# danaesavi/SocialMedia-TextImage-Classification-AuxLosses

Measured on AMD Instinct MI355X. Metric: posts/sec (fwd+bwd) Bernice+ViT-B/16 attn-fusion, bs=64, higher is better.
Workload: dtype bf16; 1 GPU; BASELINE config 2: Bernice+ViT-B/16, attention fusion, no aux loss, bs=64/GPU; step=full train step: fwd + loss + bwd + grad exchange + AdamW + weight refresh, posts_per_gpu=64, image=224, vocab=250002, parallelism=dp1, weights=random-init at true shapes

## Files before the change

### socialmedia-textimage-classification-auxlosses_amd/csrc/engine.hip

```cpp
#include <string>
#include <vector>
#include <cstdlib>
#include <cstdio>
#include "mmhip_common.h"
#include "mmhip_host.h"

using namespace mmhip;

namespace {

struct LayerOff {
    size_t qkv_w, qkv_b, ao_w, ao_b, ln1_w, ln1_b, fc1_w, fc1_b, fc2_w, fc2_b, ln2_w, ln2_b, begin, end;
};
struct LayerW16 {
    size_t qkv, ao, fc1, fc2, qkvT, aoT, fc1T, fc2T;
};
struct TextAct {
    size_t qkv, ctx, pre1, a1, u, h, pre2, out, mean1, rstd1, mean2, rstd2, lse;
    size_t a1p, outp;
};

}

struct mmhip_engine {
// ... 31 lines not shown
    int B = 0, T = 0, Bt = 0; bool itm = false, train_mode = false, fwd_done = false, bwd_begun = false;
    bool skip_itc = false, itc_done = false;
    uint64_t seed = 0;
    size_t ws_base = 0;
    int itc_max_world = 0, itc_world = 1, itc_rank = 0;
    size_t h_g_txt = 0, h_g_img = 0, h_g_rowlse = 0, h_g_collse = 0, h_g_loss = 0, h_g_dtn = 0, h_g_din = 0, h_g_ws = 0;
    bool bd_itc_global = false; float bd_w_itc = 0.f;
    const float *bd_out_cls = nullptr, *bd_logits = nullptr, *bd_out_tim = nullptr, *bd_feats = nullptr;
    hipStream_t side = nullptr;
    int vision_ready_B = 0;
    bool vit_is_long = false;
    hipStream_t side_vit[2] = {nullptr, nullptr};
    hipEvent_t ev_fork = nullptr, ev_vit = nullptr, ev_ready[2] = {nullptr, nullptr}, ev_tn[2] = {nullptr, nullptr};
    hipEvent_t ev_layer[2] = {nullptr, nullptr}, ev_opt = nullptr;
    bool tn_pending[2] = {false, false};
    bool txt_only = false;
    std::string tm_prefix = "dual_encoder.text_model.";
    size_t lin_w = 0, lin_b = 0;
    size_t tt_all = 0; bool has_tt = false;
    int cls_only = -1;
    bool cls_compact = false;
    int overlap = -1;
    int part[2] = {-1, -1}, cur_part[2] = {0, 0}; bool part_auto = false;
    int part_bwd = -1;
    int spans_on = 0; hipEvent_t span_ev[6] = {nullptr, nullptr, nullptr, nullptr, nullptr, nullptr}; bool span_set[6] = {false, false, false, false, false, false};
    int span(int i, hipStream_t s) {
        if (!spans_on) return 0;
        if (!span_ev[i]) { hipError_t r = hipEventCreate(&span_ev[i]); if (r != hipSuccess) return (int)r; }
        hipError_t r = hipEventRecord(span_ev[i], s);
        span_set[i] = r == hipSuccess;
// ... 331 lines not shown
            CHECK_HIP(hipEventRecord(ev->b, s));
            e.ev_used++;
        }
        return 0;
    }
    CHECK_RC(run_gemm(e, g0, s));
    return run_gemm(e, g1, s);
}

int side_init(mmhip_engine& e) {
    if (e.overlap < 0) { const char* v = getenv("MMHIP_OVERLAP"); e.overlap = v ? atoi(v) : 1; }
    if (!e.overlap || e.side) return 0;
    CHECK_HIP(pool_stream(POOL_SIDE, &e.side));
    CHECK_HIP(pool_stream(POOL_VIT, &e.side_vit[0]));
    CHECK_HIP(pool_stream(POOL_VIT_HI, &e.side_vit[1]));
    hipEvent_t* evs[9] = {&e.ev_fork, &e.ev_vit, &e.ev_ready[0], &e.ev_ready[1], &e.ev_tn[0], &e.ev_tn[1], &e.ev_layer[0], &e.ev_layer[1], &e.ev_opt};
    for (auto ev : evs) CHECK_HIP(hipEventCreateWithFlags(ev, hipEventDisableTiming));
    return 0;
}
inline bool use_side(const mmhip_engine& e) { return e.overlap > 0 && e.side && e.timing != 2; }

int refresh_layer(mmhip_engine& e, const float* base, const LayerOff& o, const LayerW16& w, bool transposed, hipStream_t s, int H, int I) {
    CastMat m[4] = {{base + o.qkv_w, e.ws + w.qkv, transposed ? e.ws + w.qkvT : nullptr, 3 * H, H, 0},
                    {base + o.ao_w, e.ws + w.ao, transposed ? e.ws + w.aoT : nullptr, H, H, 0},
                    {base + o.fc1_w, e.ws + w.fc1, transposed ? e.ws + w.fc1T : nullptr, I, H, 0},
                    {base + o.fc2_w, e.ws + w.fc2, transposed ? e.ws + w.fc2T : nullptr, H, I, 0}};
    CHECK_HIP(launch_cast_group(m, 4, e.px ? DT_PAIR : e.dt(), s));
    return 0;
}

int vit_forward(mmhip_engine& e, const float* pixels, hipStream_t s) {
    const mmhip_config& c = e.cfg;
    const int H = e.Hv(), I = e.Iv(), B = e.B, P = e.P(), Kpp = e.Kpp(), dt = e.dt();
    const int Mv = B * P;
    const bool clip = e.clip();
// ... 290 lines not shown
    return 0;
}

int heads_backward(mmhip_engine& e, hipStream_t s) {
    const mmhip_config& c = e.cfg;
    const int H = c.hidden, E = c.proj_dim, C = c.num_labels, T = e.T, B = e.B, Bt = e.Bt, dt = e.dt();
    const int P = e.P(), Hv = e.Hv(), ZW = H + Hv;
    const float* W = e.train;
    float* Gd = e.grad;
    const float* d_out_cls = e.bd_out_cls ? e.bd_out_cls : e.wsp<float>(e.h_d_out_cls);
    const float* d_logits = e.bd_logits;
    const float* d_out_tim = e.bd_out_tim;
    float* dfeats = e.wsp<float>(e.h_dfeats);
    float* feats = e.wsp<float>(e.h_feats);
    float* z = e.wsp<float>(e.h_z);
    float* dxcls = e.wsp<float>(e.h_dxcls);
    const DropCfg nodrop = make_drop(0.f, 0, 0, false);
    CHECK_HIP(launch_small_nn(small(d_out_cls, C, W + e.cls_w, H, nullptr, dfeats, H, B, H, C), s));
    CHECK_HIP(launch_elementwise(EW_DROPOUT, dfeats, nullptr, dfeats, (size_t)B * H, 0.f, make_drop(c.p_head, e.seed, STREAM_HEAD, e.train_mode), s));
    if (e.bd_feats) CHECK_HIP(launch_elementwise(EW_ADD, dfeats, e.bd_feats, dfeats, (size_t)B * H, 1.f, nodrop, s));
    CHECK_HIP(launch_small_tn(small(d_out_cls, C, e.wsp<float>(e.h_featd), H, nullptr, Gd + e.cls_w, H, B, H, 0, 0, 1), DT_F32, C, s));
    CHECK_HIP(launch_bias_grad_f32(d_out_cls, B, C, C, Gd + e.cls_b, 1, s));
    if (e.itm) {
        if (d_out_tim) {
            CHECK_HIP(launch_small_nn(small(d_out_tim, 2, W + e.tim_w, H, nullptr, dfeats + (size_t)B * H, H, B, H, 2), s));
            CHECK_HIP(launch_small_tn(small(d_out_tim, 2, feats + (size_t)B * H, H, nullptr, Gd + e.tim_w, H, B, H, 0, 0, 1), DT_F32, 2, s));
            CHECK_HIP(launch_bias_grad_f32(d_out_tim, B, 2, 2, Gd + e.tim_b, 1, s));
        } else {
            CHECK_HIP(hipMemsetAsync(dfeats + (size_t)B * H, 0, (size_t)B * H * 4, s));
        }
    }
    float* dpre = e.wsp<float>(e.h_dpre);
    CHECK_HIP(launch_elementwise(EW_RELU_BWD, dfeats, feats, dpre, (size_t)Bt * H, 0.f, nodrop, s));
    CHECK_HIP(launch_small_tn(small(dpre, H, z, ZW, nullptr, Gd + e.fus_w, ZW, Bt, ZW, 0, 0, 1), DT_F32, H, s));
    CHECK_HIP(launch_bias_grad_f32(dpre, Bt, H, H, Gd + e.fus_b, 1, s));
    float* dz = e.wsp<float>(e.h_dz);
    CHECK_HIP(launch_small_nn(small(dpre, H, W + e.fus_w, ZW, nullptr, dz, ZW, Bt, ZW, H), s));
    CHECK_HIP(hipMemcpy2DAsync(dxcls, (size_t)H * 4, dz, (size_t)ZW * 4, (size_t)H * 4, Bt, hipMemcpyDeviceToDevice, s));
    if (c.fusion == MMHIP_FUSION_ATTENTION) {
        const float* dctx = dz + H;
        float* q = e.wsp<float>(e.h_q);
        CHECK_HIP(launch_small_tn(small(dctx, ZW, e.wsp<float>(e.h_xbar), H, nullptr, Gd + e.fv_w, H, Bt, H, 0, 0, 1), DT_F32, H, s));
        CHECK_HIP(launch_bias_grad_f32(dctx, Bt, H, ZW, Gd + e.fv_b, 1, s));
        CHECK_HIP(launch_small_nn(small(dctx, ZW, W + e.fv_w, H, nullptr, e.wsp<float>(e.h_dxbar), H, Bt, H, H), s));
        FusionAttnBwdArgs fb{e.wsp<float>(e.h_dxbar), e.wsp<float>(e.h_prob), e.ws + e.v_out, e.wsp<float>(e.h_dqk), Bt, B, P, H, 1.0f / sqrtf((float)H)};
        CHECK_HIP(launch_fusion_attn_bwd(fb, dt, s));
        CHECK_HIP(launch_small_tn(small(q, H, e.wsp<float>(e.h_dqk), H, nullptr, Gd + e.fk_w, H, Bt, H, 0, 0, 1), DT_F32, H, s));
        CHECK_HIP(launch_small_nt(small(e.wsp<float>(e.h_dqk), H, W + e.fk_w, H, nullptr, e.wsp<float>(e.h_dq), H, Bt, H, H), DT_F32, s));
        CHECK_HIP(launch_small_tn(small(e.wsp<float>(e.h_dq), H, z, ZW, nullptr, Gd + e.fq_w, H, Bt, H, 0, 0, 1), DT_F32, H, s));
        CHECK_HIP(launch_bias_grad_f32(e.wsp<float>(e.h_dq), Bt, H, H, Gd + e.fq_b, 1, s));
        CHECK_HIP(launch_small_nn(small(e.wsp<float>(e.h_dq), H, W + e.fq_w, H, nullptr, dxcls, H, Bt, H, H, ACT_NONE, 1), s));
    }
    if (d_logits || e.bd_itc_global) {
        if (e.bd_itc_global) {
            const int G = e.itc_world * B;
            ItcGlobalBwdArgs gb{};
            gb.txt_n = e.wsp<float>(e.h_g_txt); gb.img_n = e.wsp<float>(e.h_g_img); gb.logit_scale = W + e.logit_scale;
            gb.rowlse = e.wsp<float>(e.h_g_rowlse); gb.collse = e.wsp<float>(e.h_g_collse);
            gb.txt_inv = e.wsp<float>(e.h_txt_inv); gb.img_inv = e.wsp<float>(e.h_img_inv);
            gb.d_txt_n = e.wsp<float>(e.h_g_dtn); gb.d_img_n = e.wsp<float>(e.h_g_din);
            gb.dtxt_e = e.wsp<float>(e.h_dtxt_e); gb.dimg_e = e.wsp<float>(e.h_dimg_e); gb.dlogit_scale = Gd + e.logit_scale;
            gb.ws = e.wsp<float>(e.h_g_ws); gb.G = G; gb.E = E; gb.Bl = B; gb.r0 = e.itc_rank * B;
            gb.scale = e.bd_w_itc * (float)e.itc_world / (2.f * (float)G);
            CHECK_HIP(launch_itc_global_bwd(gb, s));
        } else {
            ItcBwdArgs ib{d_logits, e.wsp<float>(e.h_logits), e.wsp<float>(e.h_txt_n), e.wsp<float>(e.h_img_n), e.wsp<float>(e.h_txt_inv),
                          e.wsp<float>(e.h_img_inv), W + e.logit_scale, e.wsp<float>(e.h_dtxt_e), e.wsp<float>(e.h_dimg_e), Gd + e.logit_scale, B, E};
            CHECK_HIP(launch_itc_bwd(ib, s));
        }
        CHECK_HIP(launch_small_tn(small(e.wsp<float>(e.h_dtxt_e), E, e.wsp<float>(e.h_tpool), H, nullptr, Gd + e.tproj_w, H, B, H, 0, 0, 1), DT_F32, E, s));
        CHECK_HIP(launch_small_tn(small(e.wsp<float>(e.h_dimg_e), E, e.wsp<float>(e.h_vpool), Hv, nullptr, Gd + e.vproj_w, Hv, B, Hv, 0, 0, 1), DT_F32, E, s));
        CHECK_HIP(launch_small_nn(small(e.wsp<float>(e.h_dtxt_e), E, W + e.tproj_w, H, nullptr, e.wsp<float>(e.h_dtpool), H, B, H, E), s));
        CHECK_HIP(launch_elementwise(EW_TANH_BWD, e.wsp<float>(e.h_dtpool), e.wsp<float>(e.h_tpool), e.wsp<float>(e.h_dprepool), (size_t)B * H, 0.f, nodrop, s));
        CHECK_HIP(launch_small_tn(small(e.wsp<float>(e.h_dprepool), H, z, ZW, nullptr, Gd + e.t_pool_w, H, B, H, 0, 0, 1), DT_F32, H, s));
        CHECK_HIP(launch_bias_grad_f32(e.wsp<float>(e.h_dprepool), B, H, H, Gd + e.t_pool_b, 1, s));
        CHECK_HIP(launch_small_nn(small(e.wsp<float>(e.h_dprepool), H, W + e.t_pool_w, H, nullptr, dxcls, H, B, H, H, ACT_NONE, 1), s));
    }
    CHECK_HIP(launch_scatter_cls_rows(dxcls, e.ws + e.g_dx, Bt, e.cls_compact ? 1 : T, H, dt, s, e.gscale()));
    return 0;
}

ClsHeadArgs txt_head_args(const mmhip_engine& e) {
    const mmhip_config& c = e.cfg;
    return cls_head(text_last(e), e.cls_compact ? (size_t)c.hidden : (size_t)e.T * c.hidden, e.dt(), e.train + e.lin_w, e.B, c.num_labels, c.hidden,
                    make_drop(c.p_head, e.seed, STREAM_HEAD, e.train_mode));
}
int txt_head_forward(mmhip_engine& e, const int64_t* onehot, const float* class_w, float* logits, float* loss, int* n_correct, hipStream_t s) {
    ClsHeadArgs a = txt_head_args(e);
    a.bias = e.train + e.lin_b; a.logits = e.wsp<float>(e.h_out_cls);
    if (onehot) {
        a.onehot = onehot; a.class_w = class_w; a.loss = e.wsp<float>(e.h_loss); a.n_correct = n_correct; a.d_logits_out = e.wsp<float>(e.h_d_out_cls);
    }
    CHECK_HIP(launch_cls_head_fwd(a, s));
// ... 108 lines not shown
        pr[1].B = e.ws + a.a1p;
        for (auto& q : pr) tn_pair(q, np);
    }
    {
        const int i = e.side && ps == e.side ? 1 : 0;
        CHECK_HIP(launch_gemm_tn(pr, 4, 0, dt, 0, ps, 1.0f / e.gscale(), e.x3_bytes[i] ? e.ws + e.x3_ws[i] : nullptr, e.x3_bytes[i]));
    }
    if (side) {
        CHECK_HIP(hipEventRecord(e.ev_tn[set], e.side));
        e.tn_pending[set] = true;
    }
    return 0;
}

int backward_finish(mmhip_engine& e, hipStream_t s) {
    for (int set = 0; set < 2; ++set)
        if (e.tn_pending[set]) {
            CHECK_HIP(hipStreamWaitEvent(s, e.ev_tn[set], 0));
            e.tn_pending[set] = false;
        }
    return 0;
}

static unsigned* g_nonfinite = nullptr;
static unsigned* g_skip = nullptr;
inline unsigned* guard_counter(const mmhip_engine& e) { return e.guard ? e.guard : g_nonfinite; }
inline unsigned* guard_flag(const mmhip_engine& e) { return e.guard ? e.guard + 1 : g_skip; }

int embed_backward(mmhip_engine& e, hipStream_t s) {
    const mmhip_config& c = e.cfg;
// ... 41 lines not shown
    if (c.txt_kind == MMHIP_TXT_BERT && c.max_pos < c.max_text_len) return MMHIP_E_INVALID;
    mmhip_engine* e = new (std::nothrow) mmhip_engine();
    if (!e) return MMHIP_E_INVALID;
    e->cfg = c;
    if (c.dtype == MMHIP_BF16X3) { const char* v = getenv("MMHIP_X3_PAIRS"); e->px = v ? atoi(v) != 0 : true; }
    if (c.dtype == MMHIP_BF16X3) { const char* v = getenv("MMHIP_X3_BWD"); const int n = v ? atoi(v) : 3; e->bwd_np = n >= 1 && n <= 3 ? n : 3; }
    build_layout(*e);
    build_workspace(*e);
    *out = e;
    return 0;
}
void mmhip_destroy(mmhip_handle h) {
    if (!h) return;
    if (h->side) {
        (void)hipStreamSynchronize(h->side);
        for (hipEvent_t ev : {h->ev_fork, h->ev_vit, h->ev_ready[0], h->ev_ready[1], h->ev_tn[0], h->ev_tn[1], h->ev_layer[0], h->ev_layer[1], h->ev_opt})
            if (ev) (void)hipEventDestroy(ev);
        for (auto sv : h->side_vit) if (sv) (void)hipStreamSynchronize(sv);
        for (auto ev : h->span_ev) if (ev) (void)hipEventDestroy(ev);
    }
    for (auto& ev : h->evs) { (void)hipEventDestroy(ev.a); (void)hipEventDestroy(ev.b); }
    delete h;
}
int mmhip_param_count(mmhip_handle h) { return h ? (int)h->params.size() : MMHIP_E_INVALID; }
int mmhip_param_info_at(mmhip_handle h, int i, mmhip_param_info* out) {
    if (!h || !out || i < 0 || i >= (int)h->params.size()) return MMHIP_E_INVALID;
    *out = h->params[i];
    return 0;
}
uint64_t mmhip_buffer_numel(mmhip_handle h, int buffer) { return !h ? 0 : (buffer == 0 ? h->n_frozen : h->n_train); }
uint64_t mmhip_workspace_bytes(mmhip_handle h) { return h ? h->ws_need : 0; }
// ... 56 lines not shown

int mmhip_forward(mmhip_handle h, const int64_t* ids, const int64_t* mask, const float* pixels, const int64_t* tim_ids,
                  const int64_t* tim_mask, int B, int T, int train, uint64_t seed, float* out_cls, float* logits_per_text,
                  float* out_tim, float* mm_features, void* stream) {
    if (!h || !h->ws || h->txt_only) return MMHIP_E_STATE;
    if (!ids || !mask || B < 1 || T < 1) return MMHIP_E_INVALID;
    if ((tim_ids == nullptr) != (tim_mask == nullptr)) return MMHIP_E_INVALID;
    mmhip_engine& e = *h;
    const bool imported = pixels == nullptr;
    if (imported && e.vision_ready_B != B) return MMHIP_E_STATE;
    e.vision_ready_B = 0;
    if (B > e.cfg.max_posts || T > e.cfg.max_text_len) return MMHIP_E_CAPACITY;
    hipStream_t s = (hipStream_t)stream;
    e.B = B; e.T = T; e.itm = tim_ids != nullptr; e.Bt = e.itm ? 2 * B : B; e.train_mode = train != 0; e.seed = seed;
    e.fwd_done = false; e.bwd_begun = false;
    const size_t nb = (size_t)B * T * 8;
    CHECK_HIP(launch_copy_ids_clamped(ids, e.wsp<int64_t>(e.ids_all), (size_t)B * T, e.cfg.vocab, e.bad_index, s));
    CHECK_HIP(hipMemcpyAsync(e.ws + e.mask_all, mask, nb, hipMemcpyDeviceToDevice, s));
    if (e.itm) {
        CHECK_HIP(launch_copy_ids_clamped(tim_ids, e.wsp<int64_t>(e.ids_all) + (size_t)B * T, (size_t)B * T, e.cfg.vocab, e.bad_index, s));
        CHECK_HIP(hipMemcpyAsync(e.ws + e.mask_all + nb, tim_mask, nb, hipMemcpyDeviceToDevice, s));
    }
    CHECK_RC(side_init(e));
    if (e.part[0] < 0) {
        e.part[0] = e.part[1] = 0; e.part_auto = true;
        if (const char* v = getenv("MMHIP_PART")) {
            int a = 0, b = 0;
            e.part_auto = false;
            if (sscanf(v, "%d,%d", &a, &b) == 2 && a > 0 && b > 0) { e.part[0] = a; e.part[1] = b; }
        }
// ... 141 lines not shown
}
int mmhip_backward_stage(mmhip_handle h, int stage, void* stream) {
    if (!h || !h->bwd_begun) return MMHIP_E_STATE;
    mmhip_engine& e = *h;
    hipStream_t s = (hipStream_t)stream;
    const int L = e.cfg.layers_txt;
    if (stage == 0) return e.txt_only ? txt_head_backward(e, s) : heads_backward(e, s);
    if (stage >= 1 && stage <= L) return text_layer_backward(e, L - stage, s);
    if (stage == L + 1) return embed_backward(e, s);
    return MMHIP_E_INVALID;
}
int mmhip_backward_join_stage(mmhip_handle h, int stage, void* stream) {
    if (!h || !h->bwd_begun) return MMHIP_E_STATE;
    mmhip_engine& e = *h;
    const int L = e.cfg.layers_txt;
    if (stage < 1 || stage > L) return 0;
    const int set = (L - stage) & 1;
    if (e.tn_pending[set]) {
        CHECK_HIP(hipStreamWaitEvent((hipStream_t)stream, e.ev_tn[set], 0));
        e.tn_pending[set] = false;
    }
    return 0;
}
int mmhip_backward_finish(mmhip_handle h, void* stream) {
    if (!h || !h->bwd_begun) return MMHIP_E_STATE;
    return backward_finish(*h, (hipStream_t)stream);
}
int mmhip_backward(mmhip_handle h, const float* d_out_cls, const float* d_logits, const float* d_out_tim, const float* d_feats, void* stream) {
    CHECK_RC(mmhip_backward_begin(h, d_out_cls, d_logits, d_out_tim, d_feats, stream));
    const int n = mmhip_num_backward_stages(h);
// ... 406 lines not shown
```

### socialmedia-textimage-classification-auxlosses_amd/csrc/gemm.hip

```cpp
#include <cstdio>
#include <cstdlib>
#include "mmhip_common.h"
#include <cstdlib>
#include <type_traits>
#include "mmhip_kernels.h"

namespace mmhip {

static constexpr int BK = 64;

template <int N> __device__ __forceinline__ void wait_vmcnt() { asm volatile("s_waitcnt vmcnt(%0)" ::"n"(N) : "memory"); }

template <int BM, int BN, int WM, int WN, int NS, int NL = 0>
struct NTCfg {
    static constexpr int NW = WM * WN, NLOAD = NL ? NL : NW, NTHR = (NW + NL) * 64;
    static constexpr int TM = BM / WM, TN = BN / WN, FM = TM / 16, FN = TN / 16;
    static constexpr int A_BYTES = BM * 128, B_BYTES = BN * 128, STAGE = A_BYTES + B_BYTES;
    static constexpr int AI = BM / 8 / NLOAD, BI = BN / 8 / NLOAD;
    static constexpr int EP_LD = TN + 4;
    static constexpr int EP_WAVE = 32 * EP_LD * 4;
    static constexpr int LDS = (NS * STAGE > NW * EP_WAVE) ? NS * STAGE : NW * EP_WAVE;
    static constexpr int BLOCKS_PER_CU = (LDS <= 80 * 1024) ? 2 : 1;
    static constexpr int LPS = AI + BI;
};
// ... 440 lines not shown
    const int lane = threadIdx.x & 63, w = threadIdx.x >> 6;
    const int r = lane & 31, h = lane >> 5;
    const int m0 = blockIdx.y * 32, n0 = blockIdx.x * 32;
    const int m = min(m0 + r, a.M - 1), n = min(n0 + r, a.N - 1);
    const TA* Ap = (const TA*)a.A + (size_t)m * a.sam;
    const float* Bp = a.W + (size_t)n * a.sbn;
    f32x16 acc = f32x16{};
    for (int k0 = w * 8 + h * 4; k0 < a.K; k0 += 8 * SG_WAVES) {
        float av[4], bv[4];
        if (a.sak == 1 && k0 + 3 < a.K && sizeof(TA) == 4 && ((((uintptr_t)(Ap + k0)) & 15) == 0)) {
            f32x4 t = *reinterpret_cast<const f32x4*>(Ap + k0);
            av[0] = t[0]; av[1] = t[1]; av[2] = t[2]; av[3] = t[3];
        } else {
#pragma unroll
            for (int e = 0; e < 4; ++e) av[e] = (k0 + e < a.K) ? (float)Ap[(size_t)(k0 + e) * a.sak] : 0.f;
        }
        if (a.sbk == 1 && k0 + 3 < a.K && ((((uintptr_t)(Bp + k0)) & 15) == 0)) {
            f32x4 t = *reinterpret_cast<const f32x4*>(Bp + k0);
            bv[0] = t[0]; bv[1] = t[1]; bv[2] = t[2]; bv[3] = t[3];
        } else {
#pragma unroll
            for (int e = 0; e < 4; ++e) bv[e] = (k0 + e < a.K) ? Bp[(size_t)(k0 + e) * a.sbk] : 0.f;
        }
#pragma unroll
        for (int e = 0; e < 4; ++e) acc = __builtin_amdgcn_mfma_f32_32x32x2f32(av[e], bv[e], acc, 0, 0, 0);
    }
#pragma unroll
    for (int reg = 0; reg < 16; ++reg) red[w][(reg & 3) + 8 * (reg >> 2) + 4 * h][r] = acc[reg];
    __syncthreads();
    for (int i = threadIdx.x; i < 32 * 32; i += SG_WAVES * 64) {
// ... 287 lines not shown
        }
    }
    flush();
    return hipGetLastError();
}

hipError_t launch_small_gemm(const SmallGemmArgs& a, int a_dtype, hipStream_t s) {
    if (a.M <= 0 || a.N <= 0) return hipSuccess;
    dim3 grid((a.N + 31) / 32, (a.M + 31) / 32);
    if (a_dtype == DT_F32) hipLaunchKernelGGL(small_gemm_kernel<float>, grid, dim3(SG_WAVES * 64), 0, s, a);
    else if (a_dtype == DT_BF16) hipLaunchKernelGGL(small_gemm_kernel<bf16_t>, grid, dim3(SG_WAVES * 64), 0, s, a);
    else hipLaunchKernelGGL(small_gemm_kernel<f16_t>, grid, dim3(SG_WAVES * 64), 0, s, a);
    return hipGetLastError();
}
hipError_t launch_small_nt(const SmallGemmArgs& a0, int a_dtype, hipStream_t s) {
    SmallGemmArgs a = a0;
    a.sam = a.lda; a.sak = 1; a.sbk = 1; a.sbn = a.ldw;
    return launch_small_gemm(a, a_dtype, s);
}
hipError_t launch_small_nn(const SmallGemmArgs& a0, hipStream_t s) {
    SmallGemmArgs a = a0;
    a.sam = a.lda; a.sak = 1; a.sbk = a.ldw; a.sbn = 1;
    return launch_small_gemm(a, DT_F32, s);
}
hipError_t launch_small_tn(const SmallGemmArgs& a0, int b_dtype, int n_rows, hipStream_t s) {
    if (b_dtype != DT_F32) return hipErrorInvalidValue;
    SmallGemmArgs a = a0;
    a.K = a0.M; a.M = n_rows;
    a.sam = 1; a.sak = a0.lda; a.sbk = a0.ldw; a.sbn = 1;
    return launch_small_gemm(a, DT_F32, s);
}

}
```

### socialmedia-textimage-classification-auxlosses_amd/csrc/mmhip_kernels.h

```cpp
#pragma once
#include <hip/hip_runtime.h>
#include <stdint.h>
#include "mmhip_common.h"

namespace mmhip {

enum { DT_BF16 = 0, DT_F16 = 1, DT_F32 = 2,
       DT_PAIR = 3 };
enum { ACT_NONE = 0, ACT_TANH = 1, ACT_RELU = 2 };

enum {
    GEMM_BIAS = 1,
    GEMM_GELU = 2,
    GEMM_RESIDUAL = 4,
    GEMM_DROPOUT = 8,
    GEMM_OUT_F32 = 16,
    GEMM_AUX_PRE = 32,
    GEMM_MUL_GELU_GRAD = 64,
    GEMM_TANH = 128,
    GEMM_QGELU = 256,
    GEMM_OUT_PAIR = 512,
    GEMM_OUT_PAIR_HI = 1024,
};
struct GemmNTArgs {
// ... 21 lines not shown
    int colsum_rows;
    int pair;
    int a_lo, b_lo;
    int nprod;
};
struct GemmTNGroup {
    GemmTNProblem p[GEMM_TN_MAX_GROUP];
    int count, accumulate;
    float alpha;
    int pair_serial;
};
struct SmallGemmArgs {
    const void* A; const float* W; const float* bias; float* out;
    int M, N, K, lda, ldw, ldo, act, accumulate;
    int sam, sak, sbk, sbn;
};
hipError_t launch_gemm_nt(const GemmNTArgs& a, int dtype, hipStream_t s);
enum { PATH_NONE = 0, PATH_GENERIC = 1, PATH_TILE = 2, PATH_DEEP = 3, PATH_SPLITK = 4, PATH_X3_DIRECT = 5, PATH_X3_SMALL = 6, PATH_X3_SPLIT = 7, PATH_X3_PAIR = 8 };
enum { TNPATH_GENERIC = 1, TNPATH_TILE = 2, TNPATH_X3_DIRECT = 4, TNPATH_X3_SPLIT = 8, TNPATH_X3_PAIR = 16 };
struct GemmPathRecord {
    int nt[8];
    int tn[8];
};
GemmPathRecord& gemm_path_record();
size_t nt_splitk_scratch_bytes(const GemmNTArgs& a, int dtype);
struct GemmTimingSink {
    struct Ev { hipEvent_t a, b; double flops; };
    Ev* evs; size_t capacity, used;
};
void gemm_timing_sink(GemmTimingSink* sink);
// ... 102 lines not shown
hipError_t launch_vit_assemble(const void* patches, const float* cls, const float* pos, void* x, int B, int P, int H, int dtype, hipStream_t s);
hipError_t launch_colsum(const void* x, int rows, int cols, int ld, float* out, int dtype, hipStream_t s, float* partial = nullptr, float alpha = 1.0f);
size_t partial_floats_rows(int rows, int width, int nvec);
size_t partial_floats_colsum(int rows, int cols);
size_t partial_floats_embed(int posts, int T, int width);
hipError_t launch_cast(const float* src, void* dst, size_t n, int dtype, hipStream_t s);
hipError_t launch_copy_ids_clamped(const int64_t* in, int64_t* out, size_t n, int64_t hi, unsigned* bad, hipStream_t s);
static constexpr int CAST_MAX_GROUP = 4;
struct CastMat { const float* src; void* dst; void* dstT; int rows, cols, tile_start; };
struct CastGroup { CastMat m[CAST_MAX_GROUP]; int count; };
hipError_t launch_cast_group(const CastMat* mats, int count, int dtype, hipStream_t s);
hipError_t launch_cast_transpose(const float* src, void* dst, int rows, int cols, int dtype, hipStream_t s);
hipError_t launch_gather_rows_f32(const void* src, size_t src_stride, float* out, int ldo, int rows, int H, int dtype, hipStream_t s);
hipError_t launch_scatter_rows16(const void* src, void* dst, int rows, size_t dst_stride, int H, int add, int dtype, hipStream_t s);
hipError_t launch_dropout16(const void* src, void* dst, size_t n, const DropCfg& d, int dtype, hipStream_t s);
hipError_t launch_scatter_cls_rows(const float* d, void* dx, int posts, int T, int H, int dtype, hipStream_t s, float scale = 1.0f);

struct FusionAttnArgs {
    const float* qk;
    const void* xv;
    float* prob;
    float* xbar;
    int Bt, B, P, H; float scale;
};
struct FusionAttnBwdArgs {
    const float* dxbar; const float* prob; const void* xv; float* dqk; int Bt, B, P, H; float scale;
};
hipError_t launch_fusion_attn_fwd(const FusionAttnArgs& a, int dtype, hipStream_t s);
hipError_t launch_fusion_attn_bwd(const FusionAttnBwdArgs& a, int dtype, hipStream_t s);

struct ItcArgs {
// ... 88 lines not shown
```

### socialmedia-textimage-classification-auxlosses_amd/csrc/rowops.hip

```cpp
#include <cstdlib>
#include <type_traits>
#include "mmhip_common.h"
#include "mmhip_kernels.h"

namespace mmhip {

static constexpr int MAXC = 4;

bool deterministic() {
    const char* e = getenv("MMHIP_DETERMINISTIC");
    return e && atoi(e) != 0;
}

template <typename T> __device__ __forceinline__ void load4(const T* p, float* v) {
    typename Vec<T>::v4 x = *reinterpret_cast<const typename Vec<T>::v4*>(p);
#pragma unroll
    for (int e = 0; e < 4; ++e) v[e] = to_f<T>(x[e]);
}
template <> __device__ __forceinline__ void load4<float>(const float* p, float* v) {
    f32x4 x = *reinterpret_cast<const f32x4*>(p);
#pragma unroll
    for (int e = 0; e < 4; ++e) v[e] = x[e];
}
template <typename T> __device__ __forceinline__ void store4(T* p, const float* v) {
// ... 697 lines not shown
    const int hc = H / 4;
    for (int idx = blockIdx.x * 256 + threadIdx.x; idx < rows * hc; idx += gridDim.x * 256) {
        const int rr = idx / hc, c = (idx % hc) * 4;
        float v[4];
        load4<T>(src + (size_t)rr * H + c, v);
        if (add) {
            float o[4];
            load4<T>(dst + (size_t)rr * dst_stride + c, o);
#pragma unroll
            for (int e = 0; e < 4; ++e) v[e] += o[e];
        }
        store4<T>(dst + (size_t)rr * dst_stride + c, v);
    }
}
template <typename T>
__global__ __launch_bounds__(256) void scatter_cls_kernel(const float* __restrict__ d, T* __restrict__ dx, int posts, int Tn, int H, float scale) {
    const int hc = H / 4;
    const size_t total = (size_t)posts * Tn * hc;
    for (size_t idx = (size_t)blockIdx.x * 256 + threadIdx.x; idx < total; idx += (size_t)gridDim.x * 256) {
        const int c = (idx % hc) * 4;
        const size_t row = idx / hc;
        float v[4] = {0.f, 0.f, 0.f, 0.f};
        if (row % Tn == 0) {
            load4<float>(d + (row / Tn) * H + c, v);
#pragma unroll
            for (int e = 0; e < 4; ++e) v[e] *= scale;
        }
        store4<T>(dx + row * H + c, v);
    }
}

template <typename T>
__global__ __launch_bounds__(256) void dropout16_kernel(const T* __restrict__ src, T* __restrict__ dst, size_t n, DropCfg d) {
    const size_t n4 = n / 4;
    for (size_t i = (size_t)blockIdx.x * 256 + threadIdx.x; i < n4; i += (size_t)gridDim.x * 256) {
        float v[4];
        load4<T>(src + i * 4, v);
        bool k0, k1, k2, k3;
        mm_keep2((uint32_t)(i * 4), d, k0, k1);
// ... 195 lines not shown
    if (!n) return hipSuccess;
    if (n % 4) return hipErrorInvalidValue;
    if (dtype == DT_BF16) hipLaunchKernelGGL(dropout16_kernel<bf16_t>, dim3(cap_grid(n / 4)), dim3(256), 0, s, (const bf16_t*)src, (bf16_t*)dst, n, d);
    else if (dtype == DT_F16) hipLaunchKernelGGL(dropout16_kernel<f16_t>, dim3(cap_grid(n / 4)), dim3(256), 0, s, (const f16_t*)src, (f16_t*)dst, n, d);
    else hipLaunchKernelGGL(dropout16_kernel<float>, dim3(cap_grid(n / 4)), dim3(256), 0, s, (const float*)src, (float*)dst, n, d);
    return hipGetLastError();
}
hipError_t launch_gather_rows_f32(const void* src, size_t src_stride, float* out, int ldo, int rows, int H, int dtype, hipStream_t s) {
    if (rows <= 0) return hipSuccess;
    if (H % 4 || ldo % 4) return hipErrorInvalidValue;
    if (dtype == DT_BF16) hipLaunchKernelGGL(gather_rows_f32_kernel<bf16_t>, dim3(cap_grid((size_t)rows * H / 4)), dim3(256), 0, s, (const bf16_t*)src, src_stride, out, ldo, rows, H);
    else if (dtype == DT_F16) hipLaunchKernelGGL(gather_rows_f32_kernel<f16_t>, dim3(cap_grid((size_t)rows * H / 4)), dim3(256), 0, s, (const f16_t*)src, src_stride, out, ldo, rows, H);
    else hipLaunchKernelGGL(gather_rows_f32_kernel<float>, dim3(cap_grid((size_t)rows * H / 4)), dim3(256), 0, s, (const float*)src, src_stride, out, ldo, rows, H);
    return hipGetLastError();
}
hipError_t launch_scatter_cls_rows(const float* d, void* dx, int posts, int T, int H, int dtype, hipStream_t s, float scale) {
    if (posts <= 0) return hipSuccess;
    const size_t total = (size_t)posts * T * (H / 4);
    if (dtype == DT_BF16) hipLaunchKernelGGL(scatter_cls_kernel<bf16_t>, dim3(cap_grid(total)), dim3(256), 0, s, d, (bf16_t*)dx, posts, T, H, scale);
    else if (dtype == DT_F16) hipLaunchKernelGGL(scatter_cls_kernel<f16_t>, dim3(cap_grid(total)), dim3(256), 0, s, d, (f16_t*)dx, posts, T, H, scale);
    else hipLaunchKernelGGL(scatter_cls_kernel<float>, dim3(cap_grid(total)), dim3(256), 0, s, d, (float*)dx, posts, T, H, scale);
    return hipGetLastError();
}

}
```

Measured before the change: 6240 posts/s.

## Offload head weight-gradient GEMMs to side stream and fuse ReLU-bwd into dz GEMM

The head backward now sends the weight- and bias-gradient small GEMMs (classifier, fusion, attention-fusion q/k/v, projection and pooler) to a side stream, forked with events and joined before the next forward, at stage 0 and in backward_finish. The critical-path dz GEMM reads dfeats directly and masks it by the ReLU output inside the small-GEMM kernel. The scatter reads CLS rows from dz with a stride, which removes the 2D memcpy into dxcls. The aim is to shorten the serial chain of tiny launches at the head of backward, at the cost of extra event syncs and a per-element branch in the GEMM inner loop.

```diff
diff --git a/socialmedia-textimage-classification-auxlosses_amd/csrc/engine.hip b/socialmedia-textimage-classification-auxlosses_amd/csrc/engine.hip
--- a/socialmedia-textimage-classification-auxlosses_amd/csrc/engine.hip
+++ b/socialmedia-textimage-classification-auxlosses_amd/csrc/engine.hip
@@ -69,6 +69,8 @@
     hipEvent_t ev_fork = nullptr, ev_vit = nullptr, ev_ready[2] = {nullptr, nullptr}, ev_tn[2] = {nullptr, nullptr};
     hipEvent_t ev_layer[2] = {nullptr, nullptr}, ev_opt = nullptr;
     bool tn_pending[2] = {false, false};
+    hipEvent_t ev_hfork = nullptr, ev_heads = nullptr;
+    bool heads_pending = false;
     bool txt_only = false;
     std::string tm_prefix = "dual_encoder.text_model.";
     size_t lin_w = 0, lin_b = 0;
@@ -430,11 +432,20 @@
     CHECK_HIP(pool_stream(POOL_SIDE, &e.side));
     CHECK_HIP(pool_stream(POOL_VIT, &e.side_vit[0]));
     CHECK_HIP(pool_stream(POOL_VIT_HI, &e.side_vit[1]));
-    hipEvent_t* evs[9] = {&e.ev_fork, &e.ev_vit, &e.ev_ready[0], &e.ev_ready[1], &e.ev_tn[0], &e.ev_tn[1], &e.ev_layer[0], &e.ev_layer[1], &e.ev_opt};
+    hipEvent_t* evs[11] = {&e.ev_fork, &e.ev_vit, &e.ev_ready[0], &e.ev_ready[1], &e.ev_tn[0], &e.ev_tn[1], &e.ev_layer[0], &e.ev_layer[1], &e.ev_opt,
+                           &e.ev_hfork, &e.ev_heads};
     for (auto ev : evs) CHECK_HIP(hipEventCreateWithFlags(ev, hipEventDisableTiming));
     return 0;
 }
 inline bool use_side(const mmhip_engine& e) { return e.overlap > 0 && e.side && e.timing != 2; }
+inline bool neck_on() { const char* v = getenv("MMHIP_NECK"); return v ? atoi(v) != 0 : true; }
+int join_heads(mmhip_engine& e, hipStream_t s) {
+    if (e.heads_pending) {
+        CHECK_HIP(hipStreamWaitEvent(s, e.ev_heads, 0));
+        e.heads_pending = false;
+    }
+    return 0;
+}
 
 int refresh_layer(mmhip_engine& e, const float* base, const LayerOff& o, const LayerW16& w, bool transposed, hipStream_t s, int H, int I) {
     CastMat m[4] = {{base + o.qkv_w, e.ws + w.qkv, transposed ? e.ws + w.qkvT : nullptr, 3 * H, H, 0},
@@ -755,42 +766,70 @@
     float* dfeats = e.wsp<float>(e.h_dfeats);
     float* feats = e.wsp<float>(e.h_feats);
     float* z = e.wsp<float>(e.h_z);
-    float* dxcls = e.wsp<float>(e.h_dxcls);
     const DropCfg nodrop = make_drop(0.f, 0, 0, false);
+    const bool neck = neck_on();
+    const bool off = neck && use_side(e);
+    hipStream_t ps = off ? e.side : s;
+    auto fork = [&]() -> int {
+        if (off) { CHECK_HIP(hipEventRecord(e.ev_hfork, s)); CHECK_HIP(hipStreamWaitEvent(e.side, e.ev_hfork, 0)); }
+        return 0;
+    };
+    CHECK_RC(join_heads(e, s));
+    auto cls_grads = [&]() -> int {
+        CHECK_HIP(launch_small_tn(small(d_out_cls, C, e.wsp<float>(e.h_featd), H, nullptr, Gd + e.cls_w, H, B, H, 0, 0, 1), DT_F32, C, ps));
+        CHECK_HIP(launch_bias_grad_f32(d_out_cls, B, C, C, Gd + e.cls_b, 1, ps));
+        return 0;
+    };
+    if (off) { CHECK_RC(fork()); CHECK_RC(cls_grads()); }
     CHECK_HIP(launch_small_nn(small(d_out_cls, C, W + e.cls_w, H, nullptr, dfeats, H, B, H, C), s));
     CHECK_HIP(launch_elementwise(EW_DROPOUT, dfeats, nullptr, dfeats, (size_t)B * H, 0.f, make_drop(c.p_head, e.seed, STREAM_HEAD, e.train_mode), s));
     if (e.bd_feats) CHECK_HIP(launch_elementwise(EW_ADD, dfeats, e.bd_feats, dfeats, (size_t)B * H, 1.f, nodrop, s));
-    CHECK_HIP(launch_small_tn(small(d_out_cls, C, e.wsp<float>(e.h_featd), H, nullptr, Gd + e.cls_w, H, B, H, 0, 0, 1), DT_F32, C, s));
-    CHECK_HIP(launch_bias_grad_f32(d_out_cls, B, C, C, Gd + e.cls_b, 1, s));
+    if (!off) CHECK_RC(cls_grads());
     if (e.itm) {
         if (d_out_tim) {
             CHECK_HIP(launch_small_nn(small(d_out_tim, 2, W + e.tim_w, H, nullptr, dfeats + (size_t)B * H, H, B, H, 2), s));
-            CHECK_HIP(launch_small_tn(small(d_out_tim, 2, feats + (size_t)B * H, H, nullptr, Gd + e.tim_w, H, B, H, 0, 0, 1), DT_F32, 2, s));
-            CHECK_HIP(launch_bias_grad_f32(d_out_tim, B, 2, 2, Gd + e.tim_b, 1, s));
+            if (off) CHECK_RC(fork());
+            CHECK_HIP(launch_small_tn(small(d_out_tim, 2, feats + (size_t)B * H, H, nullptr, Gd + e.tim_w, H, B, H, 0, 0, 1), DT_F32, 2, ps));
+            CHECK_HIP(launch_bias_grad_f32(d_out_tim, B, 2, 2, Gd + e.tim_b, 1, ps));
         } else {
             CHECK_HIP(hipMemsetAsync(dfeats + (size_t)B * H, 0, (size_t)B * H * 4, s));
         }
     }
     float* dpre = e.wsp<float>(e.h_dpre);
-    CHECK_HIP(launch_elementwise(EW_RELU_BWD, dfeats, feats, dpre, (size_t)Bt * H, 0.f, nodrop, s));
-    CHECK_HIP(launch_small_tn(small(dpre, H, z, ZW, nullptr, Gd + e.fus_w, ZW, Bt, ZW, 0, 0, 1), DT_F32, H, s));
-    CHECK_HIP(launch_bias_grad_f32(dpre, Bt, H, H, Gd + e.fus_b, 1, s));
     float* dz = e.wsp<float>(e.h_dz);
-    CHECK_HIP(launch_small_nn(small(dpre, H, W + e.fus_w, ZW, nullptr, dz, ZW, Bt, ZW, H), s));
-    CHECK_HIP(hipMemcpy2DAsync(dxcls, (size_t)H * 4, dz, (size_t)ZW * 4, (size_t)H * 4, Bt, hipMemcpyDeviceToDevice, s));
+    float* dxcls = neck ? dz : e.wsp<float>(e.h_dxcls);
+    const int ldx = neck ? ZW : H;
+    if (neck) {
+        SmallGemmArgs g = small(dfeats, H, W + e.fus_w, ZW, nullptr, dz, ZW, Bt, ZW, H);
+        g.relu_y = feats; g.ldy = H;
+        CHECK_RC(fork());
+        CHECK_HIP(launch_elementwise(EW_RELU_BWD, dfeats, feats, dpre, (size_t)Bt * H, 0.f, nodrop, ps));
+        CHECK_HIP(launch_small_tn(small(dpre, H, z, ZW, nullptr, Gd + e.fus_w, ZW, Bt, ZW, 0, 0, 1), DT_F32, H, ps));
+        CHECK_HIP(launch_bias_grad_f32(dpre, Bt, H, H, Gd + e.fus_b, 1, ps));
+        CHECK_HIP(launch_small_nn(g, s));
+    } else {
+        CHECK_HIP(launch_elementwise(EW_RELU_BWD, dfeats, feats, dpre, (size_t)Bt * H, 0.f, nodrop, s));
+        CHECK_HIP(launch_small_tn(small(dpre, H, z, ZW, nullptr, Gd + e.fus_w, ZW, Bt, ZW, 0, 0, 1), DT_F32, H, s));
+        CHECK_HIP(launch_bias_grad_f32(dpre, Bt, H, H, Gd + e.fus_b, 1, s));
+        CHECK_HIP(launch_small_nn(small(dpre, H, W + e.fus_w, ZW, nullptr, dz, ZW, Bt, ZW, H), s));
+        CHECK_HIP(hipMemcpy2DAsync(dxcls, (size_t)H * 4, dz, (size_t)ZW * 4, (size_t)H * 4, Bt, hipMemcpyDeviceToDevice, s));
+    }
     if (c.fusion == MMHIP_FUSION_ATTENTION) {
         const float* dctx = dz + H;
         float* q = e.wsp<float>(e.h_q);
-        CHECK_HIP(launch_small_tn(small(dctx, ZW, e.wsp<float>(e.h_xbar), H, nullptr, Gd + e.fv_w, H, Bt, H, 0, 0, 1), DT_F32, H, s));
-        CHECK_HIP(launch_bias_grad_f32(dctx, Bt, H, ZW, Gd + e.fv_b, 1, s));
+        if (off) CHECK_RC(fork());
+        CHECK_HIP(launch_small_tn(small(dctx, ZW, e.wsp<float>(e.h_xbar), H, nullptr, Gd + e.fv_w, H, Bt, H, 0, 0, 1), DT_F32, H, ps));
+        CHECK_HIP(launch_bias_grad_f32(dctx, Bt, H, ZW, Gd + e.fv_b, 1, ps));
         CHECK_HIP(launch_small_nn(small(dctx, ZW, W + e.fv_w, H, nullptr, e.wsp<float>(e.h_dxbar), H, Bt, H, H), s));
         FusionAttnBwdArgs fb{e.wsp<float>(e.h_dxbar), e.wsp<float>(e.h_prob), e.ws + e.v_out, e.wsp<float>(e.h_dqk), Bt, B, P, H, 1.0f / sqrtf((float)H)};
         CHECK_HIP(launch_fusion_attn_bwd(fb, dt, s));
-        CHECK_HIP(launch_small_tn(small(q, H, e.wsp<float>(e.h_dqk), H, nullptr, Gd + e.fk_w, H, Bt, H, 0, 0, 1), DT_F32, H, s));
+        if (off) CHECK_RC(fork());
+        CHECK_HIP(launch_small_tn(small(q, H, e.wsp<float>(e.h_dqk), H, nullptr, Gd + e.fk_w, H, Bt, H, 0, 0, 1), DT_F32, H, ps));
         CHECK_HIP(launch_small_nt(small(e.wsp<float>(e.h_dqk), H, W + e.fk_w, H, nullptr, e.wsp<float>(e.h_dq), H, Bt, H, H), DT_F32, s));
-        CHECK_HIP(launch_small_tn(small(e.wsp<float>(e.h_dq), H, z, ZW, nullptr, Gd + e.fq_w, H, Bt, H, 0, 0, 1), DT_F32, H, s));
-        CHECK_HIP(launch_bias_grad_f32(e.wsp<float>(e.h_dq), Bt, H, H, Gd + e.fq_b, 1, s));
-        CHECK_HIP(launch_small_nn(small(e.wsp<float>(e.h_dq), H, W + e.fq_w, H, nullptr, dxcls, H, Bt, H, H, ACT_NONE, 1), s));
+        if (off) CHECK_RC(fork());
+        CHECK_HIP(launch_small_tn(small(e.wsp<float>(e.h_dq), H, z, ZW, nullptr, Gd + e.fq_w, H, Bt, H, 0, 0, 1), DT_F32, H, ps));
+        CHECK_HIP(launch_bias_grad_f32(e.wsp<float>(e.h_dq), Bt, H, H, Gd + e.fq_b, 1, ps));
+        CHECK_HIP(launch_small_nn(small(e.wsp<float>(e.h_dq), H, W + e.fq_w, H, nullptr, dxcls, ldx, Bt, H, H, ACT_NONE, 1), s));
     }
     if (d_logits || e.bd_itc_global) {
         if (e.bd_itc_global) {
@@ -809,15 +848,21 @@
                           e.wsp<float>(e.h_img_inv), W + e.logit_scale, e.wsp<float>(e.h_dtxt_e), e.wsp<float>(e.h_dimg_e), Gd + e.logit_scale, B, E};
             CHECK_HIP(launch_itc_bwd(ib, s));
         }
-        CHECK_HIP(launch_small_tn(small(e.wsp<float>(e.h_dtxt_e), E, e.wsp<float>(e.h_tpool), H, nullptr, Gd + e.tproj_w, H, B, H, 0, 0, 1), DT_F32, E, s));
-        CHECK_HIP(launch_small_tn(small(e.wsp<float>(e.h_dimg_e), E, e.wsp<float>(e.h_vpool), Hv, nullptr, Gd + e.vproj_w, Hv, B, Hv, 0, 0, 1), DT_F32, E, s));
+        if (off) CHECK_RC(fork());
+        CHECK_HIP(launch_small_tn(small(e.wsp<float>(e.h_dtxt_e), E, e.wsp<float>(e.h_tpool), H, nullptr, Gd + e.tproj_w, H, B, H, 0, 0, 1), DT_F32, E, ps));
+        CHECK_HIP(launch_small_tn(small(e.wsp<float>(e.h_dimg_e), E, e.wsp<float>(e.h_vpool), Hv, nullptr, Gd + e.vproj_w, Hv, B, Hv, 0, 0, 1), DT_F32, E, ps));
         CHECK_HIP(launch_small_nn(small(e.wsp<float>(e.h_dtxt_e), E, W + e.tproj_w, H, nullptr, e.wsp<float>(e.h_dtpool), H, B, H, E), s));
         CHECK_HIP(launch_elementwise(EW_TANH_BWD, e.wsp<float>(e.h_dtpool), e.wsp<float>(e.h_tpool), e.wsp<float>(e.h_dprepool), (size_t)B * H, 0.f, nodrop, s));
-        CHECK_HIP(launch_small_tn(small(e.wsp<float>(e.h_dprepool), H, z, ZW, nullptr, Gd + e.t_pool_w, H, B, H, 0, 0, 1), DT_F32, H, s));
-        CHECK_HIP(launch_bias_grad_f32(e.wsp<float>(e.h_dprepool), B, H, H, Gd + e.t_pool_b, 1, s));
-        CHECK_HIP(launch_small_nn(small(e.wsp<float>(e.h_dprepool), H, W + e.t_pool_w, H, nullptr, dxcls, H, B, H, H, ACT_NONE, 1), s));
-    }
-    CHECK_HIP(launch_scatter_cls_rows(dxcls, e.ws + e.g_dx, Bt, e.cls_compact ? 1 : T, H, dt, s, e.gscale()));
+        if (off) CHECK_RC(fork());
+        CHECK_HIP(launch_small_tn(small(e.wsp<float>(e.h_dprepool), H, z, ZW, nullptr, Gd + e.t_pool_w, H, B, H, 0, 0, 1), DT_F32, H, ps));
+        CHECK_HIP(launch_bias_grad_f32(e.wsp<float>(e.h_dprepool), B, H, H, Gd + e.t_pool_b, 1, ps));
+        CHECK_HIP(launch_small_nn(small(e.wsp<float>(e.h_dprepool), H, W + e.t_pool_w, H, nullptr, dxcls, ldx, B, H, H, ACT_NONE, 1), s));
+    }
+    if (off) {
+        CHECK_HIP(hipEventRecord(e.ev_heads, e.side));
+        e.heads_pending = true;
+    }
+    CHECK_HIP(launch_scatter_cls_rows(dxcls, e.ws + e.g_dx, Bt, e.cls_compact ? 1 : T, H, dt, s, e.gscale(), ldx));
     return 0;
 }
 
@@ -956,6 +1001,7 @@
 }
 
 int backward_finish(mmhip_engine& e, hipStream_t s) {
+    CHECK_RC(join_heads(e, s));
     for (int set = 0; set < 2; ++set)
         if (e.tn_pending[set]) {
             CHECK_HIP(hipStreamWaitEvent(s, e.ev_tn[set], 0));
@@ -1027,7 +1073,8 @@
     if (!h) return;
     if (h->side) {
         (void)hipStreamSynchronize(h->side);
-        for (hipEvent_t ev : {h->ev_fork, h->ev_vit, h->ev_ready[0], h->ev_ready[1], h->ev_tn[0], h->ev_tn[1], h->ev_layer[0], h->ev_layer[1], h->ev_opt})
+        for (hipEvent_t ev : {h->ev_fork, h->ev_vit, h->ev_ready[0], h->ev_ready[1], h->ev_tn[0], h->ev_tn[1], h->ev_layer[0], h->ev_layer[1], h->ev_opt,
+                              h->ev_hfork, h->ev_heads})
             if (ev) (void)hipEventDestroy(ev);
         for (auto sv : h->side_vit) if (sv) (void)hipStreamSynchronize(sv);
         for (auto ev : h->span_ev) if (ev) (void)hipEventDestroy(ev);
@@ -1114,6 +1161,7 @@
     hipStream_t s = (hipStream_t)stream;
     e.B = B; e.T = T; e.itm = tim_ids != nullptr; e.Bt = e.itm ? 2 * B : B; e.train_mode = train != 0; e.seed = seed;
     e.fwd_done = false; e.bwd_begun = false;
+    CHECK_RC(join_heads(e, s));
     const size_t nb = (size_t)B * T * 8;
     CHECK_HIP(launch_copy_ids_clamped(ids, e.wsp<int64_t>(e.ids_all), (size_t)B * T, e.cfg.vocab, e.bad_index, s));
     CHECK_HIP(hipMemcpyAsync(e.ws + e.mask_all, mask, nb, hipMemcpyDeviceToDevice, s));
@@ -1285,6 +1333,7 @@
     if (!h || !h->bwd_begun) return MMHIP_E_STATE;
     mmhip_engine& e = *h;
     const int L = e.cfg.layers_txt;
+    if (stage == 0) return join_heads(e, (hipStream_t)stream);
     if (stage < 1 || stage > L) return 0;
     const int set = (L - stage) & 1;
     if (e.tn_pending[set]) {
diff --git a/socialmedia-textimage-classification-auxlosses_amd/csrc/gemm.hip b/socialmedia-textimage-classification-auxlosses_amd/csrc/gemm.hip
--- a/socialmedia-textimage-classification-auxlosses_amd/csrc/gemm.hip
+++ b/socialmedia-textimage-classification-auxlosses_amd/csrc/gemm.hip
@@ -478,6 +478,12 @@
         } else {
 #pragma unroll
             for (int e = 0; e < 4; ++e) av[e] = (k0 + e < a.K) ? (float)Ap[(size_t)(k0 + e) * a.sak] : 0.f;
+        }
+        if (a.relu_y) {
+            const float* Yp = a.relu_y + (size_t)m * a.ldy;
+#pragma unroll
+            for (int e = 0; e < 4; ++e)
+                if (k0 + e < a.K && !(Yp[k0 + e] > 0.f)) av[e] = 0.f;
         }
         if (a.sbk == 1 && k0 + 3 < a.K && ((((uintptr_t)(Bp + k0)) & 15) == 0)) {
             f32x4 t = *reinterpret_cast<const f32x4*>(Bp + k0);
@@ -795,6 +801,7 @@
     return hipGetLastError();
 }
 hipError_t launch_small_nt(const SmallGemmArgs& a0, int a_dtype, hipStream_t s) {
+    if (a0.relu_y && a_dtype != DT_F32) return hipErrorInvalidValue;
     SmallGemmArgs a = a0;
     a.sam = a.lda; a.sak = 1; a.sbk = 1; a.sbn = a.ldw;
     return launch_small_gemm(a, a_dtype, s);
@@ -805,7 +812,7 @@
     return launch_small_gemm(a, DT_F32, s);
 }
 hipError_t launch_small_tn(const SmallGemmArgs& a0, int b_dtype, int n_rows, hipStream_t s) {
-    if (b_dtype != DT_F32) return hipErrorInvalidValue;
+    if (b_dtype != DT_F32 || a0.relu_y) return hipErrorInvalidValue;
     SmallGemmArgs a = a0;
     a.K = a0.M; a.M = n_rows;
     a.sam = 1; a.sak = a0.lda; a.sbk = a0.ldw; a.sbn = 1;
diff --git a/socialmedia-textimage-classification-auxlosses_amd/csrc/mmhip_kernels.h b/socialmedia-textimage-classification-auxlosses_amd/csrc/mmhip_kernels.h
--- a/socialmedia-textimage-classification-auxlosses_amd/csrc/mmhip_kernels.h
+++ b/socialmedia-textimage-classification-auxlosses_amd/csrc/mmhip_kernels.h
@@ -59,6 +59,7 @@
     const void* A; const float* W; const float* bias; float* out;
     int M, N, K, lda, ldw, ldo, act, accumulate;
     int sam, sak, sbk, sbn;
+    const float* relu_y; int ldy;
 };
 hipError_t launch_gemm_nt(const GemmNTArgs& a, int dtype, hipStream_t s);
 enum { PATH_NONE = 0, PATH_GENERIC = 1, PATH_TILE = 2, PATH_DEEP = 3, PATH_SPLITK = 4, PATH_X3_DIRECT = 5, PATH_X3_SMALL = 6, PATH_X3_SPLIT = 7, PATH_X3_PAIR = 8 };
@@ -191,7 +192,7 @@
 hipError_t launch_gather_rows_f32(const void* src, size_t src_stride, float* out, int ldo, int rows, int H, int dtype, hipStream_t s);
 hipError_t launch_scatter_rows16(const void* src, void* dst, int rows, size_t dst_stride, int H, int add, int dtype, hipStream_t s);
 hipError_t launch_dropout16(const void* src, void* dst, size_t n, const DropCfg& d, int dtype, hipStream_t s);
-hipError_t launch_scatter_cls_rows(const float* d, void* dx, int posts, int T, int H, int dtype, hipStream_t s, float scale = 1.0f);
+hipError_t launch_scatter_cls_rows(const float* d, void* dx, int posts, int T, int H, int dtype, hipStream_t s, float scale = 1.0f, int ldd = 0);
 
 struct FusionAttnArgs {
     const float* qk;
diff --git a/socialmedia-textimage-classification-auxlosses_amd/csrc/rowops.hip b/socialmedia-textimage-classification-auxlosses_amd/csrc/rowops.hip
--- a/socialmedia-textimage-classification-auxlosses_amd/csrc/rowops.hip
+++ b/socialmedia-textimage-classification-auxlosses_amd/csrc/rowops.hip
@@ -735,7 +735,7 @@
     }
 }
 template <typename T>
-__global__ __launch_bounds__(256) void scatter_cls_kernel(const float* __restrict__ d, T* __restrict__ dx, int posts, int Tn, int H, float scale) {
+__global__ __launch_bounds__(256) void scatter_cls_kernel(const float* __restrict__ d, T* __restrict__ dx, int posts, int Tn, int H, float scale, int ldd) {
     const int hc = H / 4;
     const size_t total = (size_t)posts * Tn * hc;
     for (size_t idx = (size_t)blockIdx.x * 256 + threadIdx.x; idx < total; idx += (size_t)gridDim.x * 256) {
@@ -743,7 +743,7 @@
         const size_t row = idx / hc;
         float v[4] = {0.f, 0.f, 0.f, 0.f};
         if (row % Tn == 0) {
-            load4<float>(d + (row / Tn) * H + c, v);
+            load4<float>(d + (row / Tn) * ldd + c, v);
 #pragma unroll
             for (int e = 0; e < 4; ++e) v[e] *= scale;
         }
@@ -969,13 +969,15 @@
     else hipLaunchKernelGGL(gather_rows_f32_kernel<float>, dim3(cap_grid((size_t)rows * H / 4)), dim3(256), 0, s, (const float*)src, src_stride, out, ldo, rows, H);
     return hipGetLastError();
 }
-hipError_t launch_scatter_cls_rows(const float* d, void* dx, int posts, int T, int H, int dtype, hipStream_t s, float scale) {
+hipError_t launch_scatter_cls_rows(const float* d, void* dx, int posts, int T, int H, int dtype, hipStream_t s, float scale, int ldd) {
     if (posts <= 0) return hipSuccess;
+    if (!ldd) ldd = H;
+    if (ldd % 4 || ldd < H) return hipErrorInvalidValue;
     const size_t total = (size_t)posts * T * (H / 4);
-    if (dtype == DT_BF16) hipLaunchKernelGGL(scatter_cls_kernel<bf16_t>, dim3(cap_grid(total)), dim3(256), 0, s, d, (bf16_t*)dx, posts, T, H, scale);
-    else if (dtype == DT_F16) hipLaunchKernelGGL(scatter_cls_kernel<f16_t>, dim3(cap_grid(total)), dim3(256), 0, s, d, (f16_t*)dx, posts, T, H, scale);
-    else hipLaunchKernelGGL(scatter_cls_kernel<float>, dim3(cap_grid(total)), dim3(256), 0, s, d, (float*)dx, posts, T, H, scale);
-    return hipGetLastError();
-}
-
-}
+    if (dtype == DT_BF16) hipLaunchKernelGGL(scatter_cls_kernel<bf16_t>, dim3(cap_grid(total)), dim3(256), 0, s, d, (bf16_t*)dx, posts, T, H, scale, ldd);
+    else if (dtype == DT_F16) hipLaunchKernelGGL(scatter_cls_kernel<f16_t>, dim3(cap_grid(total)), dim3(256), 0, s, d, (f16_t*)dx, posts, T, H, scale, ldd);
+    else hipLaunchKernelGGL(scatter_cls_kernel<float>, dim3(cap_grid(total)), dim3(256), 0, s, d, (float*)dx, posts, T, H, scale, ldd);
+    return hipGetLastError();
+}
+
+}
```

After: 6271 posts/s (median of 6 runs). Within noise of the previous version (+0.5%).
